# yynil/RWKV_LM_EXT

Measured on AMD Instinct MI355X. Metric: WKV6 fwd+bwd tokens/sec/GPU (B=8,T=4096,C=2048) + %HBM roofline, higher is better.
Workload: dtype bf16

## Files before the change

### rwkv_lm_ext_amd/csrc/wkv6_chunk.hip

```cpp
#include <type_traits>
#include "wkv6_chunk.h"

namespace wkv6 {
namespace {

using namespace chunk;

constexpr int GRP_BYTES = NBLK * BLK_BYTES;
constexpr int CKX_BYTES = 4 * 4096;
constexpr int CONSUMER_STAGGER = 3;
constexpr int YRS = 144;
constexpr int YS_BYTES = GRP * YRS;

enum : unsigned {
    FWD_W_RAW = 1u << 0,
    FWD_STATE_ONLY = 1u << 1,
    FWD_ACC = 1u << 2,
    FWD_GN = 1u << 3,
    FWD_AFF = 1u << 4,
    FWD_CLK = 1u << 5,
    FWD_CHAIN = 1u << 6,
    FWD_VARLEN = 1u << 7,
    FWD_SLOTS = 1u << 8,
    FWD_SNAP = 1u << 9,
    FWD_SEG = 1u << 10,
};
constexpr unsigned bit(bool on, unsigned b) { return on ? b : 0u; }
struct FwdRaw {
    uint2 pr[4], pk[4], pv[4], pw[4];
    float4 pe[4];
};
template <unsigned MODE>
__device__ __forceinline__ void fwd_request_group(const ScanArgs& a, const int b, const int h, const int ntok, const int rev, const int grp, const int wv,
                                                  const int lane, FwdRaw& raw)
{
    constexpr bool W_RAW = (MODE & FWD_W_RAW) != 0, STATE_ONLY = (MODE & FWD_STATE_ONLY) != 0, AFF = (MODE & FWD_AFF) != 0;
    const int c4 = lane & 15, tq = lane >> 4;
    const long base = (long)b * a.T * a.C + (long)h * HEAD;
    const TokAddr<AFF> tok(ntok, rev != 0);
    const int C_ = a.C;
    const unsigned span = ntok > 0 ? (unsigned)(ntok - 1) * a.C : 0u;
    const unsigned nb2 = ntok > 0 ? span * 2 + 128 : 0;
    const rsrc_t rs_r = make_rsrc(reinterpret_cast<const bf16_t*>(a.r) + base, nb2), rs_k = make_rsrc(reinterpret_cast<const bf16_t*>(a.k) + base, nb2);
    const rsrc_t rs_v = make_rsrc(reinterpret_cast<const bf16_t*>(a.v) + base, nb2);
    const rsrc_t rs_w = W_RAW ? make_rsrc(reinterpret_cast<const bf16_t*>(a.w) + base, nb2)
                              : make_rsrc(reinterpret_cast<const float*>(a.w) + base, ntok > 0 ? span * 4 + 256 : 0);
#pragma unroll
    for (int tt = 0; tt < 4; ++tt) {
        const int pl = wv * BLK + 4 * tq + tt, lp = tok.lane(pl, 4 * c4, C_);
        if constexpr (!STATE_ONLY) raw.pr[tt] = buf_load8(rs_r, tok.off(grp * GRP, pl, 4 * c4, C_, REV_R, lp) * 2);
        else raw.pr[tt] = make_uint2(0u, 0u);
        raw.pk[tt] = buf_load8(rs_k, tok.off(grp * GRP, pl, 4 * c4, C_, REV_K, lp) * 2);
        raw.pv[tt] = buf_load8(rs_v, tok.off(grp * GRP, pl, 4 * c4, C_, REV_V, lp) * 2);
        if constexpr (W_RAW) raw.pw[tt] = buf_load8(rs_w, tok.off(grp * GRP, pl, 4 * c4, C_, REV_W, lp) * 2);
        else raw.pe[tt] = buf_load16f(rs_w, tok.off(grp * GRP, pl, 4 * c4, C_, REV_W, lp) * 4);
    }
}
struct FwdChain {
    int b, ntok;
    int pb;
    bool chained_in;
    bool nx_valid;
    unsigned nx_bh;
    int nx_b, nx_ntok;
    bool nx_rev, nx_use_u;
};
__device__ __forceinline__ bool fwd_hw_wave_produces(int hw) { return hw >= 4; }
template <unsigned MODE>
__device__ __forceinline__ void chunk_fwd_body(const ScanArgs& a, const unsigned slot, const unsigned sslot, FwdRaw& raw, const FwdChain& ch = FwdChain{},
                                               const SegArgs& sg = SegArgs{})
{
    constexpr bool W_RAW = (MODE & FWD_W_RAW) != 0;
    constexpr bool STATE_ONLY = (MODE & FWD_STATE_ONLY) != 0;
    constexpr bool ACC = (MODE & FWD_ACC) != 0;
    constexpr bool GN = (MODE & FWD_GN) != 0;
    constexpr bool AFF = (MODE & FWD_AFF) != 0;
    constexpr bool CLK = (MODE & FWD_CLK) != 0;
    constexpr bool CHAIN = (MODE & FWD_CHAIN) != 0;
    constexpr bool VARLEN = (MODE & FWD_VARLEN) != 0;
    constexpr bool SLOTS = (MODE & FWD_SLOTS) != 0;
    constexpr bool SNAP = (MODE & FWD_SNAP) != 0;
    constexpr bool SEG = (MODE & FWD_SEG) != 0;
    [[maybe_unused]] const bool nxvalid = ch.nx_valid, chained_in = ch.chained_in, nx_use_u = ch.nx_use_u;
    [[maybe_unused]] const unsigned nxbh = ch.nx_bh;
    [[maybe_unused]] const int nxrev = ch.nx_rev, b_known = ch.b, ntok_known = ch.ntok, nxb = ch.nx_b, nxntok = ch.nx_ntok, pb = CHAIN ? ch.pb : 0;
    extern __shared__ __attribute__((aligned(16))) char smem[];
    const int tid = threadIdx.x, lane = tid & 63;
    const SplitConst spc = split_const();
    const int hwid = __builtin_amdgcn_readfirstlane(tid >> 6);
    const int part = a.split ? (int)(slot & 1) : 0;
    const int bh = a.split ? (int)(slot >> 1) : (CLK ? (int)(slot + 0u * (unsigned)(a.B * a.H)) : (int)slot);
    int wid, cidx;
    wid = a.split ? (hwid < 2 ? 2 * part + hwid : hwid + 2) : hwid;
    cidx = hwid;
    const bool producer = wid >= 4;
    const int wv = wid & 3;
    if constexpr (SEG) {
        static_assert(VARLEN && !CHAIN && !CLK && !ACC && !GN && (STATE_ONLY ? !SLOTS : SNAP), "items: the state pass and the stateful forward");
        if (bh / a.H >= sg.n[0]) return;
    }
    const int b = CHAIN ? b_known : (a.order ? a.order[bh / a.H] : bh / a.H), h = bh % a.H;
    const long base = VARLEN ? (long)a.tok_off[b] * a.C + (long)h * HEAD : (long)b * a.T * a.C + (long)h * HEAD;
    const bf16_t* const gr_ = reinterpret_cast<const bf16_t*>(a.r) + base;
    const bf16_t* const gk_ = reinterpret_cast<const bf16_t*>(a.k) + base;
    const bf16_t* const gv_ = reinterpret_cast<const bf16_t*>(a.v) + base;
    bf16_t* const gy_ = reinterpret_cast<bf16_t*>(a.y) + base;
    int ntok = a.T;
    if constexpr (CHAIN) ntok = ntok_known;
    else if (a.lens) ntok = min(max(a.lens[b], 0), a.T);
    [[maybe_unused]] int sq_ = b, pos_ = 0, slen_ = ntok;
    if constexpr (SEG) {
        sq_ = sg.seq[b]; pos_ = sg.pos[b]; slen_ = sg.seq_lens[sq_];
        if (ntok <= 0 || (STATE_ONLY && pos_ + ntok >= slen_)) return;
    }
    [[maybe_unused]] const bool seg_last = !SEG || pos_ + ntok >= slen_;
    [[maybe_unused]] const bool seg_entry = SEG && !(pos_ == 0 && seg_last);
    [[maybe_unused]] int sslot_ = -1;
    if constexpr (SLOTS) {
        static_assert(VARLEN && !CHAIN && !CLK, "state slots: plain packed rows only");
        if (outside_len_window(a, ntok)) return;
        sslot_ = state_slot_of(a, SEG ? sq_ : b, ntok);
    }
    [[maybe_unused]] int dslot_ = sslot_;
    if constexpr (SNAP) {
        static_assert(SLOTS && !STATE_ONLY && !ACC && !GN, "snapshots: packed stateful inference only");
        dslot_ = state_slot_out_of(a, SEG ? sq_ : b, ntok, sslot_);
        if constexpr (SEG) { if (!seg_last) dslot_ = -1; }
    }
    const int ngrp = (ntok + GRP - 1) / GRP;
    const TokAddr<AFF> tok(a, b, ntok);
    const int C_ = a.C;
#ifdef WKV6_STAMP
    unsigned long long stamp_acc[6] = {0, 0, 0, 0, 0, 0}, ts0 = 0, ts1 = 0, ts2 = 0, ts3 = 0, ts4 = 0;
#endif
#ifdef WKV6_DEBUGBUF
    unsigned long long clk0 = 0, rtc0 = 0, clk1 = 0, rtc1 = 0;
    WKV6_CLK(clk0, rtc0);
#endif
    if constexpr (CLK) { if (hwid == 0) clock_stamp(a, slot, 0); }

    if (producer) {
        const int c4 = lane & 15, tq = lane >> 4;
        float uu[4] = {0.f, 0.f, 0.f, 0.f};
        if (a.use_u) io4<bf16_t>::load(reinterpret_cast<const bf16_t*>(a.u) + h * HEAD + 4 * c4, uu);
        uint2 (&pr)[4] = raw.pr, (&pk)[4] = raw.pk, (&pv)[4] = raw.pv, (&pw)[4] = raw.pw;
        float4 (&pe)[4] = raw.pe;
        float dtot[4] = {0.f, 0.f, 0.f, 0.f};
        const unsigned span = ntok > 0 ? (unsigned)(ntok - 1) * a.C : 0u;
        const rsrc_t rs_r = make_rsrc(gr_, ntok > 0 ? span * 2 + 128 : 0), rs_k = make_rsrc(gk_, ntok > 0 ? span * 2 + 128 : 0);
        const rsrc_t rs_v = make_rsrc(gv_, ntok > 0 ? span * 2 + 128 : 0);
        const rsrc_t rs_w = W_RAW ? make_rsrc(reinterpret_cast<const bf16_t*>(a.w) + base, ntok > 0 ? span * 2 + 128 : 0)
                                  : make_rsrc(reinterpret_cast<const float*>(a.w) + base, ntok > 0 ? span * 4 + 256 : 0);
        const int lp_in[4] = {tok.lane(wv * BLK + 4 * tq, 4 * c4, C_), tok.lane(wv * BLK + 4 * tq + 1, 4 * c4, C_),
                              tok.lane(wv * BLK + 4 * tq + 2, 4 * c4, C_), tok.lane(wv * BLK + 4 * tq + 3, 4 * c4, C_)};
        auto load_quad = [&](int grp, int tt) {
            {
                const int pl = wv * BLK + 4 * tq + tt;
                const unsigned ir = tok.off(grp * GRP, pl, 4 * c4, C_, REV_R, lp_in[tt]), ik = tok.off(grp * GRP, pl, 4 * c4, C_, REV_K, lp_in[tt]);
                const unsigned iv = tok.off(grp * GRP, pl, 4 * c4, C_, REV_V, lp_in[tt]), iw = tok.off(grp * GRP, pl, 4 * c4, C_, REV_W, lp_in[tt]);
                if constexpr (!STATE_ONLY) pr[tt] = buf_load8(rs_r, ir * 2);
                else pr[tt] = make_uint2(0u, 0u);
                pk[tt] = buf_load8(rs_k, ik * 2);
                pv[tt] = buf_load8(rs_v, iv * 2);
                if constexpr (W_RAW) pw[tt] = buf_load8(rs_w, iw * 2);
                else pe[tt] = buf_load16f(rs_w, iw * 4);
            }
        };
        auto load_group = [&](int grp) {
#pragma unroll
            for (int tt = 0; tt < 4; ++tt) load_quad(grp, tt);
        };
        auto prep_group = [&](int grp, int buf, const int ntok, const float (&uu)[4], auto&& request_next) {
            char* const bb = smem + buf * GRP_BYTES + wv * BLK_BYTES;
            float r[4][4], k[4][4], cs[4][4];
#pragma unroll
            for (int tt = 0; tt < 4; ++tt) {
                const bool valid = grp * GRP + wv * BLK + 4 * tq + tt < ntok;
                r[tt][0] = bf_lo(pr[tt].x); r[tt][1] = bf_hi(pr[tt].x); r[tt][2] = bf_lo(pr[tt].y); r[tt][3] = bf_hi(pr[tt].y);
                k[tt][0] = bf_lo(pk[tt].x); k[tt][1] = bf_hi(pk[tt].x); k[tt][2] = bf_lo(pk[tt].y); k[tt][3] = bf_hi(pk[tt].y);
                float lw[4];
                if constexpr (W_RAW) {
                    lw[0] = -LOG2E * exp2_fast(LOG2E * bf_lo(pw[tt].x)); lw[1] = -LOG2E * exp2_fast(LOG2E * bf_hi(pw[tt].x));
                    lw[2] = -LOG2E * exp2_fast(LOG2E * bf_lo(pw[tt].y)); lw[3] = -LOG2E * exp2_fast(LOG2E * bf_hi(pw[tt].y));
                } else {
                    lw[0] = pe[tt].x; lw[1] = pe[tt].y; lw[2] = pe[tt].z; lw[3] = pe[tt].w;
                    if (a.wkind == 2) {
#pragma unroll
                        for (int c = 0; c < 4; ++c) lw[c] = __builtin_amdgcn_logf(lw[c]);
                    } else {
#pragma unroll
                        for (int c = 0; c < 4; ++c) lw[c] *= LOG2E;
                    }
                }
#pragma unroll
                for (int c = 0; c < 4; ++c) {
                    const float l = valid ? fmaxf(lw[c], LW_MIN2) : 0.f;
                    cs[tt][c] = tt ? cs[tt - 1][c] + l : l;
                }
                if constexpr (!STATE_ONLY) {
                    float part = 0.f;
#pragma unroll
                    for (int c = 0; c < 4; ++c) part = fmaf(r[tt][c] * uu[c], k[tt][c], part);
                    part = row_sum16(part);
                    if (c4 == 0) *reinterpret_cast<float*>(bb + OFF_COEF + (4 * tq + tt) * 4) = part;
                }
                *reinterpret_cast<uint2*>(bb + A_V * ARR + (4 * tq + tt) * RSB + 8 * c4) = pv[tt];
            }
            __builtin_amdgcn_sched_barrier(0);
            request_next();
            float pre[4], c8[4], c16[4];
#pragma unroll
            for (int c = 0; c < 4; ++c) {
                float a_, b_;
                rows16(cs[3][c], a_, b_);
                float pfx = (tq & 1) ? a_ : 0.f;
                halves32(a_ + b_, a_, b_);
                pfx += (tq & 2) ? a_ : 0.f;
                pre[c] = pfx;
                c8[c] = a_;
                c16[c] = a_ + b_;
                dtot[c] += c16[c];
            }
            if (tq == 0) {
                *reinterpret_cast<float4*>(bb + OFF_E8 + 16 * c4) =
                    make_float4(exp2_fast(c8[0]), exp2_fast(c8[1]), exp2_fast(c8[2]), exp2_fast(c8[3]));
                *reinterpret_cast<float4*>(bb + OFF_E16M8 + 16 * c4) =
                    make_float4(exp2_fast(c16[0] - c8[0]), exp2_fast(c16[1] - c8[1]), exp2_fast(c16[2] - c8[2]), exp2_fast(c16[3] - c8[3]));
            }
#pragma unroll
            for (int tt = 0; tt < 4; ++tt) {
                float rh[4], kh[4];
#pragma unroll
                for (int c = 0; c < 4; ++c) {
                    const float cex = tt ? pre[c] + cs[tt - 1][c] : pre[c];
                    const float cin = pre[c] + cs[tt][c];
                    rh[c] = r[tt][c] * exp2_fast(cex - c8[c]);
                    kh[c] = k[tt][c] * exp2_fast(c8[c] - cin);
                }
                char* const row = bb + (4 * tq + tt) * RSB + 8 * c4;
                uint2 hi, lo;
                if constexpr (!STATE_ONLY) {
                    split4(rh, hi, lo, spc);
                    *reinterpret_cast<uint2*>(row + A_RH * ARR) = hi; *reinterpret_cast<uint2*>(row + A_RL * ARR) = lo;
                }
                split4(kh, hi, lo, spc);
                *reinterpret_cast<uint2*>(row + A_KH * ARR) = hi; *reinterpret_cast<uint2*>(row + A_KL * ARR) = lo;
            }
            if constexpr (!STATE_ONLY) {
                const int x = lane & 15, g = lane >> 4;
                f4v sc = {0.f, 0.f, 0.f, 0.f};
#pragma unroll
                for (int s = 0; s < 2; ++s) {
                    const int off = x * RSB + (32 * s + 8 * g) * 2;
                    const b8v kh = ld_b8(bb + A_KH * ARR + off), kl = ld_b8(bb + A_KL * ARR + off);
                    const b8v rh = ld_b8(bb + A_RH * ARR + off), rl = ld_b8(bb + A_RL * ARR + off);
                    sc = mfma32(kh, rh, sc);
                    sc = mfma32(kh, rl, sc);
                    sc = mfma32(kl, rh, sc);
                }
                const float cf = *reinterpret_cast<const float*>(bb + OFF_COEF + x * 4);
                float scm[4];
#pragma unroll
                for (int q = 0; q < 4; ++q) {
                    const int bt = 4 * g + q;
                    scm[q] = bt < x ? sc[q] : (bt == x ? cf : 0.f);
                }
                uint2 sh, sl;
                split4(scm, sh, sl, spc);
                *reinterpret_cast<uint4*>(bb + OFF_SC + lane * 16) = make_uint4(sh.x, sh.y, sl.x, sl.y);
            }
        };

        float uu_nx[4] = {0.f, 0.f, 0.f, 0.f};
        if constexpr (CHAIN) { if (nxvalid && nx_use_u) io4<bf16_t>::load(reinterpret_cast<const bf16_t*>(a.u) + (nxbh % (unsigned)a.H) * HEAD + 4 * c4, uu_nx); }
        if (!(CHAIN && chained_in)) {
            if (ngrp > 0) {
                load_group(0);
                prep_group(0, pb & 1, ntok, uu, [&]() { load_group(1); });
            }
            __syncthreads();
        }
        for (int grp = 0; grp + 1 < ngrp; ++grp) {
            WKV6_T(ts0);
#ifdef WKV6_STAMP
            asm volatile("" :: "v"(pr[0].x), "v"(pk[0].x), "v"(pv[0].x), "v"(pw[0].x), "v"(pr[3].x), "v"(pk[3].x), "v"(pv[3].x),
                         "v"(pw[3].x));
#endif
            WKV6_T(ts1);
            prep_group(grp + 1, (grp + 1 + pb) & 1, ntok, uu, [&]() { load_group(grp + 2); });
            WKV6_T(ts2);
            WKV6_T(ts3);
            __syncthreads();
            WKV6_T(ts4);
            WKV6_ACC(0, ts1, ts0); WKV6_ACC(1, ts2, ts1); WKV6_ACC(2, ts3, ts2); WKV6_ACC(3, ts4, ts3);
        }
        if constexpr (CHAIN) {
            if (nxvalid) {
                const int nxh = (int)(nxbh % (unsigned)a.H);
                fwd_request_group<MODE>(a, nxb, nxh, nxntok, nxrev, 0, wv, lane, raw);
                prep_group(0, (ngrp + pb) & 1, nxntok, uu_nx, [&]() { fwd_request_group<MODE>(a, nxb, nxh, nxntok, nxrev, 1, wv, lane, raw); });
            }
        }
        if (ngrp > 0) __syncthreads();
        if (a.dsum && tq == 0 && part == 0)
            *reinterpret_cast<float4*>(a.dsum + ((long)(b * a.H + h) * 4 + wv) * HEAD + 4 * c4) = make_float4(dtot[0], dtot[1], dtot[2], dtot[3]);
    } else {
        const int x = lane & 15, g = lane >> 4;
        f4v St[4];
#pragma unroll
        for (int it = 0; it < 4; ++it) {
            float t4[4] = {0.f, 0.f, 0.f, 0.f};
            if (SEG && !STATE_ONLY && seg_entry) {
                if constexpr (SEG) io4<float>::load(sg.sin + ((long)b * a.H + h) * HEAD * HEAD + (long)(16 * wv + x) * HEAD + tile_ch(it) + 8 * g, t4);
            } else if (SLOTS ? sslot_ >= 0 : a.s0 != nullptr) {
                const long so_ = (long)(SLOTS ? sslot_ : b) * a.s0_bstride + ((long)h * HEAD + 16 * wv + x) * HEAD + tile_ch(it) + 8 * g;
                if (a.state_f32) io4<float>::load(reinterpret_cast<const float*>(a.s0) + so_, t4);
                else io4<bf16_t>::load(reinterpret_cast<const bf16_t*>(a.s0) + so_, t4);
            }
            St[it] = f4v{t4[0], t4[1], t4[2], t4[3]};
            asm volatile("" : "+v"(St[it]));
        }
        int troff = (4 * g + (x >> 2)) * RSB + 8 * (x & 3);
        int trow = (4 * g + (x >> 2)) * RSB + 16 * (x & 3);
        const rsrc_t rs_y = make_rsrc(a.y ? gy_ : nullptr, (!STATE_ONLY && a.y && ntok > 0) ? (unsigned)(ntok - 1) * a.C * 2u + 128u : 0u);
        const unsigned nst = VARLEN ? (unsigned)ngrp : ((unsigned)a.T + CKPT_TOK - 1) / CKPT_TOK;
        const int segs = a.ckpt_segs > 1 ? a.ckpt_segs : 1;
        const long ck_slot0 = VARLEN ? (long)h * a.ck_stride + a.ck_off[b] : ((long)((b / segs) * a.H + h) * segs + b % segs) * nst;
        const rsrc_t rs_ck = make_rsrc(a.ckpt ? a.ckpt + ck_slot0 * (HEAD * HEAD) : nullptr, a.ckpt ? nst * 16384u : 0u);
        const unsigned ystr = a.side_compact ? (unsigned)HEAD : (unsigned)a.C;
        const unsigned ych = a.side_compact ? 16u * (unsigned)cidx : 16u * (unsigned)wv;
        const rsrc_t rs_yf = make_rsrc(a.y_f32 ? a.y_f32 + (a.side_compact ? (long)sslot * a.T * HEAD : base) : nullptr,
                                       (a.y_f32 && !STATE_ONLY && ntok > 0) ? (unsigned)(ntok - 1) * ystr * 4u + 256u : 0u);
        const int lp_y = tok.lane(x, 16 * wv + 4 * g, C_), lp_ys = tok.lane(x, (int)ych + 4 * g, (int)ystr);
        [[maybe_unused]] uint4 acc_cur[NBLK] = {}, acc_nxt[NBLK] = {};
        auto acc_request = [&](int grp_, uint4 (&dst)[NBLK]) {
#pragma unroll
            for (int blk = 0; blk < NBLK; ++blk) {
                const unsigned idx = tok.off(grp_ * GRP + blk * BLK, x, 16 * wv + 4 * g, C_, REV_Y, lp_y);
                if (a.y_f32) {
                    const float4 t = buf_load16f(rs_yf, tok.off(grp_ * GRP + blk * BLK, x, (int)ych + 4 * g, (int)ystr, REV_Y, lp_ys) * 4u);
                    dst[blk] = make_uint4(__float_as_uint(t.x), __float_as_uint(t.y), __float_as_uint(t.z), __float_as_uint(t.w));
                } else {
                    const uint2 t = buf_load8(rs_y, idx * 2u);
                    dst[blk] = make_uint4(t.x, t.y, 0u, 0u);
                }
            }
        };
        auto acc_add = [&](const uint4& r, float (&o)[4]) {
            if (a.y_f32) { o[0] += __uint_as_float(r.x); o[1] += __uint_as_float(r.y); o[2] += __uint_as_float(r.z); o[3] += __uint_as_float(r.w); }
            else { o[0] += bf_lo(r.x); o[1] += bf_hi(r.x); o[2] += bf_lo(r.y); o[3] += bf_hi(r.y); }
        };
        if constexpr (ACC) {
            acc_request(0, acc_cur);
#pragma unroll
            for (int blk = 0; blk < NBLK; ++blk) asm volatile("" : "+v"(acc_cur[blk].x), "+v"(acc_cur[blk].y), "+v"(acc_cur[blk].z), "+v"(acc_cur[blk].w));
        }
        float gn_y[NBLK][4], gn_ga[4] = {1.f, 1.f, 1.f, 1.f}, gn_be[4] = {0.f, 0.f, 0.f, 0.f};
        uint2 gn_g[NBLK];
        unsigned gn_off[NBLK];
        char* const gn_stat = smem + 2 * GRP_BYTES;
        char* const ckx = smem + 2 * GRP_BYTES + (GN ? 4096 : 0) + cidx * 4096;
        char* const ys = smem + 2 * GRP_BYTES + (GN ? 4096 : 0) + CKX_BYTES;
        const int ylsh = a.split ? 2 : 3;
        auto stage_y = [&](int grp_, int blk, uint2 yb) {
            *reinterpret_cast<uint2*>(ys + (grp_ & 1) * YS_BYTES + (BLK * blk + x) * YRS + 32 * cidx + 8 * g) = yb;
        };
        const int fl_chunk = lane & ((1 << ylsh) - 1);
        const int fl_row[2] = {(GRP >> (ylsh - 1)) * cidx + (lane >> ylsh), (GRP >> (ylsh - 1)) * cidx + (64 >> ylsh) + (lane >> ylsh)};
        const int lp_fl[2] = {tok.lane(fl_row[0], 32 * part + 8 * fl_chunk, C_), tok.lane(fl_row[1], 32 * part + 8 * fl_chunk, C_)};
        auto flush_y = [&](int grp_) {
#pragma unroll
            for (int i = 0; i < 2; ++i) {
                const int row = fl_row[i], chunk = fl_chunk;
                const uint4 v = *reinterpret_cast<const uint4*>(ys + (grp_ & 1) * YS_BYTES + row * YRS + 16 * chunk);
                const unsigned off = tok.off(grp_ * GRP, row, 32 * part + 8 * chunk, C_, REV_Y, lp_fl[i]) * 2u;
                buf_store16(rs_y, off, v);
            }
        };
        const unsigned gn_bytes = (GN && ntok > 0) ? (unsigned)(ntok - 1) * a.C * 2u + 128u : 0u;
        const rsrc_t rs_gate = make_rsrc(GN ? reinterpret_cast<const bf16_t*>(a.gn_gate) + base : nullptr, gn_bytes);
        const rsrc_t rs_out = make_rsrc(GN ? reinterpret_cast<bf16_t*>(a.gn_out) + base : nullptr, gn_bytes);
        if constexpr (GN) {
            io4<bf16_t>::load(reinterpret_cast<const bf16_t*>(a.gn_gamma) + h * HEAD + 16 * wv + 4 * g, gn_ga);
            io4<bf16_t>::load(reinterpret_cast<const bf16_t*>(a.gn_beta) + h * HEAD + 16 * wv + 4 * g, gn_be);
        }
        auto gn_finish = [&](int grp) {
            const char* const st = gn_stat + (grp & 1) * 2048;
#pragma unroll
            for (int blk = 0; blk < NBLK; ++blk) {
                float s1 = 0.f, s2 = 0.f;
#pragma unroll
                for (int ww = 0; ww < 4; ++ww) {
                    const float2 t = *reinterpret_cast<const float2*>(st + ((ww * NBLK + blk) * 16 + x) * 8);
                    s1 += t.x; s2 += t.y;
                }
                const float mean = s1 * (1.f / 64.f);
                const float var = fmaxf(fmaf(-mean, mean, s2 * (1.f / 64.f)), 0.f);
                const float rstd = rsqrtf(var + a.gn_eps);
                const float gt[4] = {bf_lo(gn_g[blk].x), bf_hi(gn_g[blk].x), bf_lo(gn_g[blk].y), bf_hi(gn_g[blk].y)};
                float o[4];
#pragma unroll
                for (int qq = 0; qq < 4; ++qq) o[qq] = fmaf((gn_y[blk][qq] - mean) * rstd, gn_ga[qq], gn_be[qq]) * gt[qq];
                buf_store8(rs_out, gn_off[blk], make_uint2(pack_bf2(o[0], o[1]), pack_bf2(o[2], o[3])));
                const int p = grp * GRP + blk * BLK + x;
                if (a.gn_stats && wv == 0 && g == 0 && p < ntok) {
                    float* const sp = a.gn_stats + (((long)b * a.T + tok.token(p, REV_Y)) * a.H + h) * 2;
                    sp[0] = mean; sp[1] = rstd;
                }
            }
        };
        [[maybe_unused]] SnapPlan snaps{0, 0};
        [[maybe_unused]] int snap_j = 0, snap_at = 0;
        if constexpr (SNAP && !SEG) {
            snaps = snap_plan(a, b, ntok);
            snap_at = a.snap_every / GRP;
        }
        if constexpr (SNAP && SEG) {
            snaps = snap_plan(a, sq_, slen_);
            if (snaps.count > 0) {
                snap_j = pos_ / a.snap_every;
                snap_at = ((snap_j + 1) * a.snap_every - pos_) / GRP;
            }
        }
        if (!(CHAIN && chained_in)) __syncthreads();
        constexpr bool STAGE_Y = !STATE_ONLY && !GN;
        const bool staged = STAGE_Y && (ACC || !a.y_f32);
        for (int grp = 0; grp < ngrp; ++grp) {
            WKV6_T(ts0);
            for (int i_ = 0; i_ < cidx; ++i_) __builtin_amdgcn_s_sleep(CONSUMER_STAGGER);
            if (staged && grp > 0) flush_y(grp - 1);
            if constexpr (ACC) acc_request(grp + 1, acc_nxt);

            constexpr bool unrolled = GN || ACC;
            const int nb = unrolled ? NBLK : min(NBLK, (ntok - grp * GRP + BLK - 1) / BLK);
            constexpr int unroll_by = unrolled ? NBLK : 1;
#pragma unroll unroll_by
            for (int blk = 0; blk < nb; ++blk) {
                const char* const bb = smem + ((grp + pb) & 1) * GRP_BYTES + blk * BLK_BYTES;
                typedef unsigned v4u __attribute__((ext_vector_type(4)));
                v4u ckd[4];
                int ck_off = -1;
                if (a.ckpt && blk == 0) {
                    const unsigned st = (unsigned)grp;
#pragma unroll
                    for (int it = 0; it < 4; ++it)
#pragma unroll
                        for (int q = 0; q < 4; ++q)
                            *reinterpret_cast<float*>(ckx + ((x ^ (q << 2)) + 16 * (g & 1) + 256 * (g >> 1) + 64 * (q & 1) + 128 * (q >> 1)
                                                             + 32 * (it & 1) + 512 * (it >> 1)) * 4) = St[it][q];
#pragma unroll
                    for (int wb = 0; wb < 4; ++wb)
                        ckd[wb] = *reinterpret_cast<const v4u*>(ckx + (4 * ((g >> 1) ^ (x & 1)) + 8 * ((g & 1) ^ ((x >> 1) & 1)) + 16 * ((x >> 3) & 1)
                                                                       + 32 * ((x >> 2) & 1) + 64 * (x & 1) + 128 * ((x >> 1) & 1) + 256 * wb) * 4);
                    ck_off = (int)(st * 16384u + (((2 * (wv >> 1) + (g >> 1)) * 64 + 16 * (2 * (wv & 1) + (g & 1)) + x) * 16));
                }
                const s4v vf4 = tr_read(bb + A_V * ARR + troff + 32 * wv);
                const b8v vf = __builtin_bit_cast(b8v, __builtin_shufflevector(vf4, vf4, 0, 1, 2, 3, 4, 5, 6, 7));
                [[maybe_unused]] uint4 scp = {};
                [[maybe_unused]] float4 pm0[2] = {}, pm1[2] = {};
                [[maybe_unused]] b8v pzh[2] = {}, pzl[2] = {};
#pragma unroll
                for (int s = 0; s < 2; ++s) {
                    pm0[s] = *reinterpret_cast<const float4*>(bb + OFF_E8 + (32 * s + 8 * g) * 4);
                    pm1[s] = *reinterpret_cast<const float4*>(bb + OFF_E8 + (32 * s + 8 * g + 4) * 4);
                }
                if constexpr (!STATE_ONLY) {
                    scp = *reinterpret_cast<const uint4*>(bb + OFF_SC + lane * 16);
#pragma unroll
                    for (int s = 0; s < 2; ++s) {
                        const int off = x * RSB + (32 * s + 8 * g) * 2;
                        pzh[s] = ld_b8(bb + A_RH * ARR + off);
                        pzl[s] = ld_b8(bb + A_RL * ARR + off);
                    }
                }
                b8v pk8[4];
                float4 pdm[4];
#pragma unroll
                for (int it = 0; it < 4; ++it) {
                    pk8[it] = __builtin_bit_cast(b8v, __builtin_shufflevector(tr_read(bb + A_KH * ARR + trow + tile_tr(it)),
                                                                              tr_read(bb + A_KL * ARR + trow + tile_tr(it)), 0, 1, 2, 3, 4, 5, 6, 7));
                    pdm[it] = *reinterpret_cast<const float4*>(bb + OFF_E16M8 + (tile_ch(it) + 8 * g) * 4);
                }
                __builtin_amdgcn_sched_barrier(0);
                f4v Tt[4];
#pragma unroll
                for (int s = 0; s < 2; ++s) {
                    const float4 m0 = pm0[s], m1 = pm1[s];
                    Tt[2 * s] = f4v{St[2 * s][0] * m0.x, St[2 * s][1] * m0.y, St[2 * s][2] * m0.z, St[2 * s][3] * m0.w};
                    Tt[2 * s + 1] = f4v{St[2 * s + 1][0] * m1.x, St[2 * s + 1][1] * m1.y, St[2 * s + 1][2] * m1.z, St[2 * s + 1][3] * m1.w};
                }
                if constexpr (!STATE_ONLY) {
                    f4v yt = {0.f, 0.f, 0.f, 0.f};
                    yt = mfma32(vf, __builtin_bit_cast(b8v, scp), yt);
#pragma unroll
                    for (int s = 0; s < 2; ++s) {
                        const float t0[4] = {Tt[2 * s][0], Tt[2 * s][1], Tt[2 * s][2], Tt[2 * s][3]};
                        const float t1[4] = {Tt[2 * s + 1][0], Tt[2 * s + 1][1], Tt[2 * s + 1][2], Tt[2 * s + 1][3]};
                        uint2 h0, l0, h1, l1;
                        split4(t0, h0, l0, spc);
                        split4(t1, h1, l1, spc);
                        const b8v s_hi = __builtin_bit_cast(b8v, make_uint4(h0.x, h0.y, h1.x, h1.y));
                        const b8v s_lo = __builtin_bit_cast(b8v, make_uint4(l0.x, l0.y, l1.x, l1.y));
                        const b8v zh = pzh[s], zl = pzl[s];
                        yt = mfma32(s_hi, zh, yt);
                        yt = mfma32(s_hi, zl, yt);
                        yt = mfma32(s_lo, zh, yt);
                    }
                    {
                        const int p = grp * GRP + blk * BLK + x;
                        float o[4] = {yt[0], yt[1], yt[2], yt[3]};
                        if (!ACC && !a.y_f32) {
                            const unsigned off = tok.off(grp * GRP + blk * BLK, x, 16 * wv + 4 * g, C_, REV_Y, lp_y) * 2u;
                            const uint2 yb = make_uint2(pack_bf2(o[0], o[1]), pack_bf2(o[2], o[3]));
                            if constexpr (GN) buf_store8(rs_y, off, yb);
                            else stage_y(grp, blk, yb);
                            if constexpr (GN) {
                                const float yr[4] = {bf_lo(yb.x), bf_hi(yb.x), bf_lo(yb.y), bf_hi(yb.y)};
                                gn_off[blk] = off;
                                gn_g[blk] = buf_load8(rs_gate, off);
                                float s1 = 0.f, s2 = 0.f;
#pragma unroll
                                for (int qq = 0; qq < 4; ++qq) { gn_y[blk][qq] = yr[qq]; s1 += yr[qq]; s2 = fmaf(yr[qq], yr[qq], s2); }
                                const float two[4] = {s1, s2, 0.f, 0.f};
                                const float red = col_reduce(two);
                                if ((g & 1) == 0)
                                    *reinterpret_cast<float*>(gn_stat + (grp & 1) * 2048 + ((wv * NBLK + blk) * 16 + x) * 8 + (g >> 1) * 4) = red;
                            }
                        } else {
                            if constexpr (ACC) acc_add(acc_cur[blk], o);
                            if (!ACC && a.y_f32) buf_store16f(rs_yf, tok.off(grp * GRP + blk * BLK, x, (int)ych + 4 * g, (int)ystr, REV_Y, lp_ys) * 4u, o);
                            else stage_y(grp, blk, make_uint2(pack_bf2(o[0], o[1]), pack_bf2(o[2], o[3])));
                        }
                    }
                }
#pragma unroll
                for (int it = 0; it < 4; ++it) {
                    const f4v o = mfma32(pk8[it], vf, Tt[it]);
                    const float4 dm = pdm[it];
                    St[it][0] = dm.x * o[0];
                    St[it][1] = dm.y * o[1];
                    St[it][2] = dm.z * o[2];
                    St[it][3] = dm.w * o[3];
                }
                if (ck_off >= 0) {
#pragma unroll
                    for (int wb = 0; wb < 4; ++wb)
                        __builtin_amdgcn_raw_buffer_store_b128(ckd[wb], rs_ck, ck_off + wb * 4096, 0, 2 );
                }
            }
            if constexpr (ACC) {
#pragma unroll
                for (int blk = 0; blk < NBLK; ++blk) acc_cur[blk] = acc_nxt[blk];
            }
            WKV6_T(ts1);
            __syncthreads();
            WKV6_T(ts2);
            WKV6_ACC(0, ts1, ts0); WKV6_ACC(1, ts2, ts1);
            if constexpr (GN) gn_finish(grp);
            if constexpr (SNAP) {
                if (snap_j < snaps.count && grp + 1 == snap_at) {
                    const int ss = snap_slot_of(a, snaps, snap_j);
                    if (ss >= 0) {
                        const long so_ = ((long)ss * a.H + h) * HEAD * HEAD + (long)(16 * wv + x) * HEAD + 8 * g;
#pragma unroll
                        for (int it = 0; it < 4; ++it) {
                            const float t4[4] = {St[it][0], St[it][1], St[it][2], St[it][3]};
                            io4<float>::store(reinterpret_cast<float*>(a.s_out) + so_ + tile_ch(it), t4);
                        }
                    }
                    ++snap_j;
                    snap_at += a.snap_every / GRP;
                }
            }
        }
        if (staged && ngrp > 0) flush_y(ngrp - 1);
        if (SLOTS ? (SNAP ? dslot_ : sslot_) >= 0 : a.s_out != nullptr) {
            const long so_ = ((long)(SLOTS ? (SNAP ? dslot_ : sslot_) : b) * a.H + h) * HEAD * HEAD + (long)(16 * wv + x) * HEAD + 8 * g;
#pragma unroll
            for (int it = 0; it < 4; ++it) {
                const float t4[4] = {St[it][0], St[it][1], St[it][2], St[it][3]};
                if (a.state_f32) io4<float>::store(reinterpret_cast<float*>(a.s_out) + so_ + tile_ch(it), t4);
                else io4<bf16_t>::store(reinterpret_cast<bf16_t*>(a.s_out) + so_ + tile_ch(it), t4);
            }
        }
        if constexpr (CHAIN) {
#pragma unroll
            for (int tt = 0; tt < 4; ++tt) {
                asm volatile("" : "=v"(raw.pr[tt].x), "=v"(raw.pr[tt].y), "=v"(raw.pk[tt].x), "=v"(raw.pk[tt].y),
                                  "=v"(raw.pv[tt].x), "=v"(raw.pv[tt].y), "=v"(raw.pw[tt].x), "=v"(raw.pw[tt].y));
                asm volatile("" : "=v"(raw.pe[tt].x), "=v"(raw.pe[tt].y), "=v"(raw.pe[tt].z), "=v"(raw.pe[tt].w));
            }
        }
    }
#ifdef WKV6_DEBUGBUF
    WKV6_CLK(clk1, rtc1);
    if (a.aux && lane == 0) {
        unsigned long long* const d = reinterpret_cast<unsigned long long*>(a.aux) + ((long)bh * 16 + wid) * 8;
#ifdef WKV6_STAMP
        for (int i = 0; i < 6; ++i) d[i] = stamp_acc[i];
#else
        d[5] = (unsigned long long)__builtin_amdgcn_s_getreg((31 << 11) | 4) | ((unsigned long long)hwid << 32);
#endif
        d[6] = clk1 - clk0;
        d[7] = rtc1 - rtc0;
    }
#endif
    if constexpr (CLK) { if (hwid == 0) clock_stamp(a, slot, 1); }
    if (!STATE_ONLY && !ACC && a.zero_tail) {
        const float z[4] = {0.f, 0.f, 0.f, 0.f};
        for (int t = ntok + (tid >> 4); part == 0 && t < a.T; t += (int)(blockDim.x >> 4))
            io4<bf16_t>::store(gy_ + (unsigned)(t * a.C + 4 * (tid & 15)), z);
    }
}

template <bool W_RAW, bool STATE_ONLY, bool ACC, bool GN, bool AFF>
__global__ __launch_bounds__(512) void chunk_fwd_kernel(const ScanArgs a)
{
    FwdRaw raw;
    chunk_fwd_body<bit(W_RAW, FWD_W_RAW) | bit(STATE_ONLY, FWD_STATE_ONLY) | bit(ACC, FWD_ACC) | bit(GN, FWD_GN) | bit(AFF, FWD_AFF) |
                   bit(!STATE_ONLY && !ACC && !GN, FWD_CLK)>(a, blockIdx.x, 0u, raw);
}

template <bool W_RAW, bool STATE_ONLY>
__global__ __launch_bounds__(512) void chunk_fwd_varlen_kernel(const ScanArgs a)
{
    FwdRaw raw;
    chunk_fwd_body<bit(W_RAW, FWD_W_RAW) | bit(STATE_ONLY, FWD_STATE_ONLY) | FWD_AFF | FWD_VARLEN>(a, blockIdx.x, 0u, raw);
}

__global__ __launch_bounds__(512) void chunk_fwd_varlen_slots_kernel(const ScanArgs a)
{
    FwdRaw raw;
    chunk_fwd_body<FWD_AFF | FWD_VARLEN | FWD_SLOTS>(a, blockIdx.x, 0u, raw);
}

__global__ __launch_bounds__(512) void chunk_fwd_varlen_snap_kernel(const ScanArgs a)
{
    FwdRaw raw;
    chunk_fwd_body<FWD_AFF | FWD_VARLEN | FWD_SLOTS | FWD_SNAP>(a, blockIdx.x, 0u, raw);
}

__global__ __launch_bounds__(512) void chunk_fwd_varlen_seg_state_kernel(const ScanArgs a, const SegArgs sg)
{
    FwdRaw raw;
    chunk_fwd_body<FWD_STATE_ONLY | FWD_AFF | FWD_VARLEN | FWD_SEG>(a, blockIdx.x, 0u, raw, FwdChain{}, sg);
}
__global__ __launch_bounds__(512) void chunk_fwd_varlen_seg_kernel(const ScanArgs a, const SegArgs sg)
{
    FwdRaw raw;
    chunk_fwd_body<FWD_AFF | FWD_VARLEN | FWD_SLOTS | FWD_SNAP | FWD_SEG>(a, blockIdx.x, 0u, raw, FwdChain{}, sg);
}

template <bool W_RAW, bool STATE_ONLY>
__global__ __launch_bounds__(512) void chunk_fwd_varlen_rev_kernel(const ScanArgs a)
{
    FwdRaw raw;
    chunk_fwd_body<bit(W_RAW, FWD_W_RAW) | bit(STATE_ONLY, FWD_STATE_ONLY) | FWD_VARLEN>(a, blockIdx.x, 0u, raw);
}

template <bool W_RAW>
__global__ __launch_bounds__(512) void chunk_fwd_varlen_pair_kernel(const ScanArgs a0, const ScanArgs a1)
{
    const unsigned n = (unsigned)(a0.B * a0.H);
    const bool second = blockIdx.x >= n;
    FwdRaw raw;
    chunk_fwd_body<bit(W_RAW, FWD_W_RAW) | FWD_VARLEN>(second ? a1 : a0, second ? blockIdx.x - n : blockIdx.x, 0u, raw);
}

template <bool W_RAW>
__global__ __launch_bounds__(512) void chunk_fwd_pair_kernel(const ScanArgs a0, const ScanArgs a1)
{
    const unsigned n = (unsigned)(a0.B * a0.H);
    const bool second = blockIdx.x >= n;
    FwdRaw raw;
    chunk_fwd_body<bit(W_RAW, FWD_W_RAW)>(second ? a1 : a0, second ? blockIdx.x - n : blockIdx.x, 0u, raw);
}

template <bool W_RAW>
__global__ __launch_bounds__(512) void chunk_fwd_bi_kernel(const ScanArgs a1_, float* const ckpt2)
{
    const unsigned n = (unsigned)(a1_.B * a1_.H);
    const int H_ = a1_.H, T_ = a1_.T, use_u_ = a1_.use_u;
    const int* const order_ = a1_.order;
    const int* const lens_ = a1_.lens;
    FwdRaw raw;
    const bool producer_wave = fwd_hw_wave_produces((int)(threadIdx.x >> 6));
    const auto row_of = [&](unsigned it) { return it * gridDim.x + ((it & 1) ? gridDim.x - 1 - blockIdx.x : blockIdx.x); };
    const auto lookup = [&](unsigned row, int& b, int& ntok) {
        b = 0; ntok = 0;
        if (row < n) {
            b = order_ ? order_[row / H_] : (int)(row / H_);
            ntok = lens_ ? min(max(lens_[b], 0), T_) : T_;
        }
    };
    int b_cur, ntok_cur;
    lookup(row_of(0), b_cur, ntok_cur);
    int pb = 0;
    bool chained = false;
    for (unsigned it = 0; it * gridDim.x < n; ++it) {
        const unsigned row = row_of(it);
        if (row >= n) continue;
        const unsigned row_nx = row_of(it + 1);
        int b_nx, ntok_nx;
        lookup(row_nx, b_nx, ntok_nx);
        const int ngrp_cur = (ntok_cur + GRP - 1) / GRP;
        {
            ScanArgs a1;
            load_kernargs(a1);
            chunk_fwd_body<bit(W_RAW, FWD_W_RAW) | FWD_AFF | FWD_CHAIN>(a1, row, blockIdx.x, raw,
                                                                         FwdChain{b_cur, ntok_cur, pb, chained, true, row, b_cur, ntok_cur, true, false});
        }
        pb = (pb + ngrp_cur) & 1;
        if (!producer_wave) __builtin_amdgcn_fence(__ATOMIC_RELEASE, "workgroup");
        __syncthreads();
        if (!producer_wave) __builtin_amdgcn_fence(__ATOMIC_ACQUIRE, "workgroup");
        {
            ScanArgs a2;
            load_kernargs(a2);
            a2.reverse = 1; a2.use_u = 0; a2.accumulate = 1; a2.zero_tail = 0; a2.ckpt = ckpt2;
            chunk_fwd_body<bit(W_RAW, FWD_W_RAW) | FWD_ACC | FWD_AFF | FWD_CHAIN>(a2, row, blockIdx.x, raw,
                                                                                   FwdChain{b_cur, ntok_cur, pb, true, row_nx < n, row_nx, b_nx, ntok_nx, false, use_u_ != 0});
        }
        pb = (pb + ngrp_cur) & 1;
        chained = true;
        __syncthreads();
        b_cur = b_nx; ntok_cur = ntok_nx;
    }
}

constexpr size_t FWD_LDS = 2 * (size_t)GRP_BYTES + CKX_BYTES + 2 * YS_BYTES;

template <bool W_RAW, bool STATE_ONLY, bool ACC, bool GN, bool AFF> hipError_t launch_fwd_variant2(const ScanArgs& a, hipStream_t st)
{
    constexpr auto K = chunk_fwd_kernel<W_RAW, STATE_ONLY, ACC, GN, AFF>;
    constexpr size_t lds = FWD_LDS + (GN ? 4096 : 0);
    return a.split ? launch<K>(dim3(2 * a.B * a.H), dim3(384), lds, st, a) : launch<K>(dim3(a.B * a.H), dim3(512), lds, st, a);
}
template <bool W_RAW, bool STATE_ONLY, bool ACC, bool GN = false> hipError_t launch_fwd_variant(const ScanArgs& a, hipStream_t st)
{
    if constexpr (!ACC && !GN) { if (a.rev_n) return launch_fwd_variant2<W_RAW, STATE_ONLY, false, false, false>(a, st); }
    else if (a.rev_n) return hipErrorNotSupported;
    return launch_fwd_variant2<W_RAW, STATE_ONLY, ACC, GN, true>(a, st);
}

}

hipError_t launch_chunk_fwd(const ScanArgs& a_, hipStream_t st)
{
    if (!offsets_fit(a_)) return hipErrorInvalidValue;
    ScanArgs a = a_;
    a.split = want_split(a.B * a.H);
    a.clk = clock_claim(0, &a.clk_slots);
    attach_debug_buffer(a);
    const bool raw = a.wkind == 1;
    if (a.gn_out) {
        if (a.split || a.accumulate || a.y_f32 || a.zero_tail) return hipErrorNotSupported;
        return raw ? launch_fwd_variant<true, false, false, true>(a, st) : launch_fwd_variant<false, false, false, true>(a, st);
    }
    if (a.accumulate) return raw ? launch_fwd_variant<true, false, true>(a, st) : launch_fwd_variant<false, false, true>(a, st);
    return raw ? launch_fwd_variant<true, false, false>(a, st) : launch_fwd_variant<false, false, false>(a, st);
}

hipError_t launch_chunk_fwd_pair(const ScanArgs& a0_, const ScanArgs& a1_, hipStream_t st)
{
    if (!offsets_fit(a0_) || !offsets_fit(a1_)) return hipErrorInvalidValue;
    if (!same_problem(a0_, a1_)) return hipErrorInvalidValue;
    const auto plain = [](const ScanArgs& a) { return !a.accumulate && !a.y_f32 && !a.zero_tail && !a.gn_out && !a.dsum && !a.ckpt_segs; };
    if (!plain(a0_) || !plain(a1_)) return hipErrorNotSupported;
    if (want_split(a0_.B * a0_.H)) {
        if (hipError_t e = launch_chunk_fwd(a0_, st)) return e;
        return launch_chunk_fwd(a1_, st);
    }
    ScanArgs a0 = a0_, a1 = a1_;
    a0.split = a1.split = 0;
    const dim3 grid(2 * a0.B * a0.H);
    return a0.wkind == 1 ? launch<chunk_fwd_pair_kernel<true>>(grid, dim3(512), FWD_LDS, st, a0, a1)
                         : launch<chunk_fwd_pair_kernel<false>>(grid, dim3(512), FWD_LDS, st, a0, a1);
}

hipError_t launch_chunk_fwd_bi(const ScanArgs& a1_, const ScanArgs& a2_, int* slots, hipStream_t st)
{
    const int n = bi_slots(a1_.B * a1_.H);
    if (slots) *slots = n;
    if (!n || !a1_.y_f32 || a1_.gn_out || a1_.dsum || a1_.ckpt_segs) return hipErrorNotSupported;
    if (!offsets_fit(a1_)) return hipErrorInvalidValue;
    ScanArgs a1 = a1_, a2 = a2_;
    a1.split = a2.split = 0;
    a1.side_compact = a2.side_compact = 1;
    attach_debug_buffer(a1);
    attach_debug_buffer(a2);
    return a1.wkind == 1 ? launch<chunk_fwd_bi_kernel<true>>(dim3(n), dim3(512), FWD_LDS, st, a1, a2.ckpt)
                         : launch<chunk_fwd_bi_kernel<false>>(dim3(n), dim3(512), FWD_LDS, st, a1, a2.ckpt);
}

template <bool W_RAW, bool STATE_ONLY> static hipError_t launch_fwd_varlen_inst(const ScanArgs& a, hipStream_t st)
{
    const dim3 grid(a.B * a.H);
    return a.rev_n ? launch<chunk_fwd_varlen_rev_kernel<W_RAW, STATE_ONLY>>(grid, dim3(512), FWD_LDS, st, a)
                   : launch<chunk_fwd_varlen_kernel<W_RAW, STATE_ONLY>>(grid, dim3(512), FWD_LDS, st, a);
}
static bool varlen_fwd_plain(const ScanArgs& a)
{
    return !(a.reverse || a.accumulate || a.y_f32 || a.zero_tail || a.gn_out || a.dsum || a.ckpt_segs > 1 || a.side_compact);
}
hipError_t launch_chunk_fwd_varlen(const ScanArgs& a_, bool state_only, hipStream_t st)
{
    if (!offsets_fit(a_) || !packed_arrays_ok(a_)) return hipErrorInvalidValue;
    if (!varlen_fwd_plain(a_)) return hipErrorNotSupported;
    const ScanArgs a = packed_launch_args(a_);
    const bool raw = a.wkind == 1;
    if (state_only) return raw ? launch_fwd_varlen_inst<true, true>(a, st) : launch_fwd_varlen_inst<false, true>(a, st);
    return raw ? launch_fwd_varlen_inst<true, false>(a, st) : launch_fwd_varlen_inst<false, false>(a, st);
}

hipError_t launch_chunk_fwd_slots(const ScanArgs& a_, hipStream_t st)
{
    if (!offsets_fit(a_) || !packed_arrays_ok(a_) || !slots_ok(a_) || a_.wkind != 2) return hipErrorInvalidValue;
    if (!varlen_fwd_plain(a_) || a_.rev_n || a_.ckpt) return hipErrorNotSupported;
// ... 51 lines not shown
```

### rwkv_lm_ext_amd/csrc/wkv6_common.h

```cpp
#pragma once
#include <hip/hip_runtime.h>
#include <stdint.h>

namespace wkv6 {

constexpr int HEAD = 64;

typedef unsigned short bf16_t;
typedef _Float16 f16_t;

__device__ __forceinline__ float bf_lo(uint32_t x) { return __uint_as_float(x << 16); }
__device__ __forceinline__ float bf_hi(uint32_t x) { return __uint_as_float(x & 0xffff0000u); }
__device__ __forceinline__ uint32_t pack_bf2(float lo, float hi)
{
    typedef __bf16 bf2 __attribute__((ext_vector_type(2)));
    typedef float f2 __attribute__((ext_vector_type(2)));
    f2 v = {lo, hi};
    bf2 h = __builtin_convertvector(v, bf2);
    return __builtin_bit_cast(uint32_t, h);
}

typedef __amdgpu_buffer_rsrc_t rsrc_t;
__device__ __forceinline__ rsrc_t make_rsrc(const void* base, unsigned bytes)
{
    return __builtin_amdgcn_make_buffer_rsrc(const_cast<void*>(base), 0, (int)bytes, 0x00020000);
}
__device__ __forceinline__ uint2 buf_load8(rsrc_t r, unsigned off)
{
    typedef unsigned v2u __attribute__((ext_vector_type(2)));
    const v2u v = __builtin_amdgcn_raw_buffer_load_b64(r, (int)off, 0, 0);
    return make_uint2(v.x, v.y);
}
__device__ __forceinline__ float4 buf_load16f(rsrc_t r, unsigned off)
{
    typedef unsigned v4u __attribute__((ext_vector_type(4)));
    const v4u v = __builtin_amdgcn_raw_buffer_load_b128(r, (int)off, 0, 0);
    return make_float4(__uint_as_float(v.x), __uint_as_float(v.y), __uint_as_float(v.z), __uint_as_float(v.w));
}
__device__ __forceinline__ void buf_store16f(rsrc_t r, unsigned off, const float (&v)[4])
{
    typedef unsigned v4u __attribute__((ext_vector_type(4)));
    __builtin_amdgcn_raw_buffer_store_b128(v4u{__float_as_uint(v[0]), __float_as_uint(v[1]), __float_as_uint(v[2]), __float_as_uint(v[3])},
                                           r, (int)off, 0, 0);
}
__device__ __forceinline__ void buf_store16(rsrc_t r, unsigned off, uint4 v)
{
    typedef unsigned v4u __attribute__((ext_vector_type(4)));
    __builtin_amdgcn_raw_buffer_store_b128(v4u{v.x, v.y, v.z, v.w}, r, (int)off, 0, 0);
}
__device__ __forceinline__ void buf_store8(rsrc_t r, unsigned off, uint2 v)
{
    typedef unsigned v2u __attribute__((ext_vector_type(2)));
    __builtin_amdgcn_raw_buffer_store_b64(v2u{v.x, v.y}, r, (int)off, 0, 0);
}

template <typename T> struct io4;
template <> struct io4<bf16_t> {
    static __device__ __forceinline__ void load(const bf16_t* p, float (&o)[4])
    {
        const uint2 raw = *reinterpret_cast<const uint2*>(p);
        o[0] = bf_lo(raw.x); o[1] = bf_hi(raw.x); o[2] = bf_lo(raw.y); o[3] = bf_hi(raw.y);
    }
    static __device__ __forceinline__ void store(bf16_t* p, const float (&v)[4])
    {
        uint2 raw; raw.x = pack_bf2(v[0], v[1]); raw.y = pack_bf2(v[2], v[3]);
        *reinterpret_cast<uint2*>(p) = raw;
    }
};
template <> struct io4<f16_t> {
    typedef f16_t h4 __attribute__((ext_vector_type(4)));
    static __device__ __forceinline__ void load(const f16_t* p, float (&o)[4])
    {
        const h4 raw = *reinterpret_cast<const h4*>(p);
        o[0] = (float)raw[0]; o[1] = (float)raw[1]; o[2] = (float)raw[2]; o[3] = (float)raw[3];
    }
    static __device__ __forceinline__ void store(f16_t* p, const float (&v)[4])
    {
        const h4 raw = {(f16_t)v[0], (f16_t)v[1], (f16_t)v[2], (f16_t)v[3]};
        *reinterpret_cast<h4*>(p) = raw;
    }
};
template <> struct io4<float> {
    static __device__ __forceinline__ void load(const float* p, float (&o)[4])
    {
        const float4 raw = *reinterpret_cast<const float4*>(p);
        o[0] = raw.x; o[1] = raw.y; o[2] = raw.z; o[3] = raw.w;
    }
    static __device__ __forceinline__ void store(float* p, const float (&v)[4])
    {
        *reinterpret_cast<float4*>(p) = make_float4(v[0], v[1], v[2], v[3]);
    }
};

template <typename T, int CPT> struct ion;
template <typename T> struct ion<T, 4> : io4<T> {};
template <> struct ion<bf16_t, 2> {
    static __device__ __forceinline__ void load(const bf16_t* p, float (&o)[2])
    {
        const uint32_t raw = *reinterpret_cast<const uint32_t*>(p);
        o[0] = bf_lo(raw); o[1] = bf_hi(raw);
    }
    static __device__ __forceinline__ void store(bf16_t* p, const float (&v)[2])
    {
        *reinterpret_cast<uint32_t*>(p) = pack_bf2(v[0], v[1]);
    }
    static __device__ __forceinline__ float load1(const bf16_t* p) { return bf_lo((uint32_t)*p); }
};
template <> struct ion<f16_t, 2> {
// ... 139 lines not shown
```

Before: 57.46 million.

## Load v directly into LDS via buffer_load LDS-DMA in plain forward kernel

For the dense, unsplit plain forward kernel, v is no longer loaded into registers and then written to LDS. It now goes straight into a swizzled, unpadded LDS layout using buffer_load_dwordx4 with the lds modifier, one group ahead, and the transpose read offsets are adapted to match. The per-group __syncthreads is replaced by explicit vmcnt/lgkmcnt waits plus s_barrier, and the consumer stagger is reduced. A separate register-path kernel is kept for split and f32-y launches. This is meant to cut VGPR pressure and the VALU/LDS-store work for v, at the cost of fragile hand-tuned waitcnt counts and m0 manipulation in inline asm.

```diff
diff --git a/rwkv_lm_ext_amd/csrc/wkv6_chunk.hip b/rwkv_lm_ext_amd/csrc/wkv6_chunk.hip
--- a/rwkv_lm_ext_amd/csrc/wkv6_chunk.hip
+++ b/rwkv_lm_ext_amd/csrc/wkv6_chunk.hip
@@ -9,8 +9,11 @@
 constexpr int GRP_BYTES = NBLK * BLK_BYTES;
 constexpr int CKX_BYTES = 4 * 4096;
 constexpr int CONSUMER_STAGGER = 3;
+constexpr int CONSUMER_STAGGER_VDMA = 1;
 constexpr int YRS = 144;
 constexpr int YS_BYTES = GRP * YRS;
+constexpr int VROW = 2 * HEAD;
+static_assert(BLK * VROW <= ARR && (8 * VROW) == 64 * 16, "the unpadded v rows of a block keep A_V's place in the operand image");
 
 enum : unsigned {
     FWD_W_RAW = 1u << 0,
@@ -24,6 +27,7 @@
     FWD_SLOTS = 1u << 8,
     FWD_SNAP = 1u << 9,
     FWD_SEG = 1u << 10,
+    FWD_VDMA = 1u << 11,
 };
 constexpr unsigned bit(bool on, unsigned b) { return on ? b : 0u; }
 struct FwdRaw {
@@ -81,6 +85,8 @@
     constexpr bool SLOTS = (MODE & FWD_SLOTS) != 0;
     constexpr bool SNAP = (MODE & FWD_SNAP) != 0;
     constexpr bool SEG = (MODE & FWD_SEG) != 0;
+    constexpr bool VDMA = (MODE & FWD_VDMA) != 0;
+    static_assert(!VDMA || (AFF && !STATE_ONLY && !ACC && !GN && !CHAIN && !VARLEN), "LDS-DMA of v: the dense plain kernel (launched unsplit) only");
     [[maybe_unused]] const bool nxvalid = ch.nx_valid, chained_in = ch.chained_in, nx_use_u = ch.nx_use_u;
     [[maybe_unused]] const unsigned nxbh = ch.nx_bh;
     [[maybe_unused]] const int nxrev = ch.nx_rev, b_known = ch.b, ntok_known = ch.ntok, nxb = ch.nx_b, nxntok = ch.nx_ntok, pb = CHAIN ? ch.pb : 0;
@@ -161,7 +167,7 @@
                 if constexpr (!STATE_ONLY) pr[tt] = buf_load8(rs_r, ir * 2);
                 else pr[tt] = make_uint2(0u, 0u);
                 pk[tt] = buf_load8(rs_k, ik * 2);
-                pv[tt] = buf_load8(rs_v, iv * 2);
+                if constexpr (!VDMA) pv[tt] = buf_load8(rs_v, iv * 2);
                 if constexpr (W_RAW) pw[tt] = buf_load8(rs_w, iw * 2);
                 else pe[tt] = buf_load16f(rs_w, iw * 4);
             }
@@ -204,7 +210,7 @@
                     part = row_sum16(part);
                     if (c4 == 0) *reinterpret_cast<float*>(bb + OFF_COEF + (4 * tq + tt) * 4) = part;
                 }
-                *reinterpret_cast<uint2*>(bb + A_V * ARR + (4 * tq + tt) * RSB + 8 * c4) = pv[tt];
+                if constexpr (!VDMA) *reinterpret_cast<uint2*>(bb + A_V * ARR + (4 * tq + tt) * RSB + 8 * c4) = pv[tt];
             }
             __builtin_amdgcn_sched_barrier(0);
             request_next();
@@ -283,8 +289,8 @@
         for (int grp = 0; grp + 1 < ngrp; ++grp) {
             WKV6_T(ts0);
 #ifdef WKV6_STAMP
-            asm volatile("" :: "v"(pr[0].x), "v"(pk[0].x), "v"(pv[0].x), "v"(pw[0].x), "v"(pr[3].x), "v"(pk[3].x), "v"(pv[3].x),
-                         "v"(pw[3].x));
+            asm volatile("" :: "v"(pr[0].x), "v"(pk[0].x), "v"(pw[0].x), "v"(pr[3].x), "v"(pk[3].x), "v"(pw[3].x));
+            if constexpr (!VDMA) asm volatile("" :: "v"(pv[0].x), "v"(pv[3].x));
 #endif
             WKV6_T(ts1);
             prep_group(grp + 1, (grp + 1 + pb) & 1, ntok, uu, [&]() { load_group(grp + 2); });
@@ -321,6 +327,9 @@
             asm volatile("" : "+v"(St[it]));
         }
         int troff = (4 * g + (x >> 2)) * RSB + 8 * (x & 3);
+        [[maybe_unused]] const auto v_swz = [](int t) { return 2 * ((t >> 1) & 3); };
+        const int v_col = VDMA ? 0 : 32 * wv;
+        if constexpr (VDMA) troff = (4 * g + (x >> 2)) * VROW + 16 * ((2 * wv + ((x & 3) >> 1)) ^ v_swz(4 * g + (x >> 2))) + 8 * (x & 1);
         int trow = (4 * g + (x >> 2)) * RSB + 16 * (x & 3);
         const rsrc_t rs_y = make_rsrc(a.y ? gy_ : nullptr, (!STATE_ONLY && a.y && ntok > 0) ? (unsigned)(ntok - 1) * a.C * 2u + 128u : 0u);
         const unsigned nst = VARLEN ? (unsigned)ngrp : ((unsigned)a.T + CKPT_TOK - 1) / CKPT_TOK;
@@ -422,13 +431,39 @@
                 snap_at = ((snap_j + 1) * a.snap_every - pos_) / GRP;
             }
         }
+        [[maybe_unused]] const rsrc_words_t rw_v = make_rsrc_words(gv_, (VDMA && ntok > 0) ? (unsigned)(ntok - 1) * a.C * 2u + 128u : 0u);
+        [[maybe_unused]] const unsigned v_lds = (unsigned)__builtin_amdgcn_readfirstlane(
+            (int)(unsigned)(unsigned long)(__attribute__((address_space(3))) char*)smem + wv * BLK_BYTES + A_V * ARR);
+        [[maybe_unused]] int lp_vd[2] = {0, 0};
+        if constexpr (VDMA) {
+#pragma unroll
+            for (int i = 0; i < 2; ++i) {
+                const int row = 8 * i + (lane >> 3);
+                lp_vd[i] = tok.lane(wv * BLK + row, 8 * ((lane & 7) ^ v_swz(row)), C_);
+            }
+        }
+        auto v_dma = [&](int grp_) {
+#pragma unroll
+            for (int i = 0; i < 2; ++i)
+                buf_load16_lds(rw_v, tok.off(grp_ * GRP, wv * BLK + 8 * i + (lane >> 3), 0, C_, REV_V, lp_vd[i]) * 2u,
+                               v_lds + (unsigned)((grp_ & 1) * GRP_BYTES + i * 8 * VROW));
+        };
+        if constexpr (VDMA) {
+#pragma unroll
+            for (int i = 0; i < 4; ++i)
+                *reinterpret_cast<uint4*>(smem + (i >> 1) * GRP_BYTES + wv * BLK_BYTES + A_V * ARR + (i & 1) * 8 * VROW + 16 * lane) = make_uint4(0u, 0u, 0u, 0u);
+            asm volatile("s_waitcnt lgkmcnt(0)" ::: "memory");
+            v_dma(0);
+            asm volatile("s_waitcnt vmcnt(0)" ::: "memory");
+        }
         if (!(CHAIN && chained_in)) __syncthreads();
         constexpr bool STAGE_Y = !STATE_ONLY && !GN;
-        const bool staged = STAGE_Y && (ACC || !a.y_f32);
+        const bool staged = STAGE_Y && (VDMA || ACC || !a.y_f32);
         for (int grp = 0; grp < ngrp; ++grp) {
             WKV6_T(ts0);
-            for (int i_ = 0; i_ < cidx; ++i_) __builtin_amdgcn_s_sleep(CONSUMER_STAGGER);
-            if (staged && grp > 0) flush_y(grp - 1);
+            for (int i_ = 0; i_ < cidx; ++i_) __builtin_amdgcn_s_sleep(VDMA ? CONSUMER_STAGGER_VDMA : CONSUMER_STAGGER);
+            if constexpr (VDMA) v_dma(grp + 1);
+            if (staged && (VDMA || grp > 0)) flush_y(grp - 1);
             if constexpr (ACC) acc_request(grp + 1, acc_nxt);
 
             constexpr bool unrolled = GN || ACC;
@@ -454,7 +489,7 @@
                                                                        + 32 * ((x >> 2) & 1) + 64 * (x & 1) + 128 * ((x >> 1) & 1) + 256 * wb) * 4);
                     ck_off = (int)(st * 16384u + (((2 * (wv >> 1) + (g >> 1)) * 64 + 16 * (2 * (wv & 1) + (g & 1)) + x) * 16));
                 }
-                const s4v vf4 = tr_read(bb + A_V * ARR + troff + 32 * wv);
+                const s4v vf4 = tr_read(bb + A_V * ARR + troff + v_col);
                 const b8v vf = __builtin_bit_cast(b8v, __builtin_shufflevector(vf4, vf4, 0, 1, 2, 3, 4, 5, 6, 7));
                 [[maybe_unused]] uint4 scp = {};
                 [[maybe_unused]] float4 pm0[2] = {}, pm1[2] = {};
@@ -509,7 +544,7 @@
                     {
                         const int p = grp * GRP + blk * BLK + x;
                         float o[4] = {yt[0], yt[1], yt[2], yt[3]};
-                        if (!ACC && !a.y_f32) {
+                        if (!ACC && (VDMA || !a.y_f32)) {
                             const unsigned off = tok.off(grp * GRP + blk * BLK, x, 16 * wv + 4 * g, C_, REV_Y, lp_y) * 2u;
                             const uint2 yb = make_uint2(pack_bf2(o[0], o[1]), pack_bf2(o[2], o[3]));
                             if constexpr (GN) buf_store8(rs_y, off, yb);
@@ -553,7 +588,11 @@
                 for (int blk = 0; blk < NBLK; ++blk) acc_cur[blk] = acc_nxt[blk];
             }
             WKV6_T(ts1);
-            __syncthreads();
+            if constexpr (VDMA) {
+                if (a.ckpt) asm volatile("s_waitcnt vmcnt(6)" ::: "memory");
+                else asm volatile("s_waitcnt vmcnt(2)" ::: "memory");
+                asm volatile("s_waitcnt lgkmcnt(0)\n\ts_barrier" ::: "memory");
+            } else __syncthreads();
             WKV6_T(ts2);
             WKV6_ACC(0, ts1, ts0); WKV6_ACC(1, ts2, ts1);
             if constexpr (GN) gn_finish(grp);
@@ -613,12 +652,20 @@
     }
 }
 
+template <bool STATE_ONLY, bool ACC, bool GN, bool AFF> constexpr bool fwd_plain_affine = !STATE_ONLY && !ACC && !GN && AFF;
+
 template <bool W_RAW, bool STATE_ONLY, bool ACC, bool GN, bool AFF>
 __global__ __launch_bounds__(512) void chunk_fwd_kernel(const ScanArgs a)
 {
     FwdRaw raw;
     chunk_fwd_body<bit(W_RAW, FWD_W_RAW) | bit(STATE_ONLY, FWD_STATE_ONLY) | bit(ACC, FWD_ACC) | bit(GN, FWD_GN) | bit(AFF, FWD_AFF) |
-                   bit(!STATE_ONLY && !ACC && !GN, FWD_CLK)>(a, blockIdx.x, 0u, raw);
+                   bit(!STATE_ONLY && !ACC && !GN, FWD_CLK) | bit(fwd_plain_affine<STATE_ONLY, ACC, GN, AFF>, FWD_VDMA)>(a, blockIdx.x, 0u, raw);
+}
+template <bool W_RAW>
+__global__ __launch_bounds__(512) void chunk_fwd_vregs_kernel(const ScanArgs a)
+{
+    FwdRaw raw;
+    chunk_fwd_body<bit(W_RAW, FWD_W_RAW) | FWD_AFF | FWD_CLK>(a, blockIdx.x, 0u, raw);
 }
 
 template <bool W_RAW, bool STATE_ONLY>
@@ -734,6 +781,11 @@
 {
     constexpr auto K = chunk_fwd_kernel<W_RAW, STATE_ONLY, ACC, GN, AFF>;
     constexpr size_t lds = FWD_LDS + (GN ? 4096 : 0);
+    if constexpr (fwd_plain_affine<STATE_ONLY, ACC, GN, AFF>) {
+        constexpr auto KR = chunk_fwd_vregs_kernel<W_RAW>;
+        if (a.split) return launch<KR>(dim3(2 * a.B * a.H), dim3(384), lds, st, a);
+        if (a.y_f32) return launch<KR>(dim3(a.B * a.H), dim3(512), lds, st, a);
+    }
     return a.split ? launch<K>(dim3(2 * a.B * a.H), dim3(384), lds, st, a) : launch<K>(dim3(a.B * a.H), dim3(512), lds, st, a);
 }
 template <bool W_RAW, bool STATE_ONLY, bool ACC, bool GN = false> hipError_t launch_fwd_variant(const ScanArgs& a, hipStream_t st)
diff --git a/rwkv_lm_ext_amd/csrc/wkv6_common.h b/rwkv_lm_ext_amd/csrc/wkv6_common.h
--- a/rwkv_lm_ext_amd/csrc/wkv6_common.h
+++ b/rwkv_lm_ext_amd/csrc/wkv6_common.h
@@ -24,6 +24,19 @@
 __device__ __forceinline__ rsrc_t make_rsrc(const void* base, unsigned bytes)
 {
     return __builtin_amdgcn_make_buffer_rsrc(const_cast<void*>(base), 0, (int)bytes, 0x00020000);
+}
+typedef unsigned rsrc_words_t __attribute__((ext_vector_type(4)));
+__device__ __forceinline__ rsrc_words_t make_rsrc_words(const void* base, unsigned bytes)
+{
+    const unsigned long p = reinterpret_cast<unsigned long>(base);
+    return rsrc_words_t{(unsigned)__builtin_amdgcn_readfirstlane((int)(unsigned)p), (unsigned)__builtin_amdgcn_readfirstlane((int)((unsigned)(p >> 32) & 0xffffu)),
+                        (unsigned)__builtin_amdgcn_readfirstlane((int)bytes), 0x00020000u};
+}
+__device__ __forceinline__ void buf_load16_lds(rsrc_words_t r, unsigned off, unsigned lds_base)
+{
+    unsigned keep;
+    asm volatile("s_nop 4\n\ts_mov_b32 %0, m0\n\ts_mov_b32 m0, %3\n\ts_nop 0\n\tbuffer_load_dwordx4 %1, %2, 0 offen lds\n\ts_mov_b32 m0, %0"
+                 : "=&s"(keep) : "v"(off), "s"(r), "s"(lds_base) : "memory");
 }
 __device__ __forceinline__ uint2 buf_load8(rsrc_t r, unsigned off)
 {
```

Result: no change. 57.95 million (median of 6 runs) (+0.8%).
